# wyysf-98/MoCo_Flow

Hardware: AMD Instinct MI355X
Metric: ray-samples/sec (4096 rays x 64 samples) (higher is better)
Workload: dtype f32; 1 GPU; C2 NeRF 8x256 fp32 4096x64; rays_per_gpu=4096, samples_per_ray=64, global_rays=4096, loss_allreduce=False, main_has_collective=False

## Files before the change

### moco_flow_amd/csrc/mf_layout.hpp

```cpp
#pragma once
#include "../../include/mocoflow_hip.h"
#include "mf_core.hpp"

namespace mf {

inline int64_t round_up(int64_t x, int64_t m) { return (x + m - 1) / m * m; }

inline int single_skip_layer(uint32_t skip_mask, int D) {
  int s = 0;
  for (int l = 1; l < D; ++l)
    if ((skip_mask >> l) & 1u) { if (s) return -1; s = l; }
  return s;
}

constexpr int kPackHidden = -1;
struct PackBlock {
  const float* src;
  int s_n, s_k;
  int kind;
  int steps;
  int split;
  int cols;
};

struct PackRegion {
  PackBlock blk[2];
  int tiles;
  int groups;
  int n_rows;
  int row_terms;
  long long dst_group0;
};

struct ResCopy { const float* src; int dst_off; int n; float scale = 1.f; };

struct PackJob {
  PackRegion reg[MF_MAX_LAYERS + 3];
  int n_regions;
  int bf16;
  int xyz_cols;
  int half;
  float wscale;
  long long total_groups;
  float* panels;
  float* poison;
  ResCopy res[2];
  int n_res, res_floats;
  float* resident;
  PackRegion& add(int tiles, int groups, const PackBlock& b0, const PackBlock& b1 = PackBlock{}) {
    PackRegion& R = reg[n_regions++];
    R = PackRegion{{b0, b1}, tiles, groups, 0, 0, total_groups};
    total_groups += (long long)groups * tiles;
    return R;
  }
};
static_assert(sizeof(PackJob) <= 2048, "pack_panels_kernel's argument block");

int launch_pack(const PackJob& job, hipStream_t st, const char* what);

inline bool nerf_layout(const mf_nerf_desc& d, NetLayout& L, int bf16 = 0) {
  L = NetLayout{};
  const bool x3 = bf16 == MF_PREC_BF16X3;
  L.bf16 = bf16 ? 1 : 0;
  if (d.W != 256 && d.W != 128) return false;
  if (d.D < 2 || d.D + 1 > MF_MAX_LAYERS) return false;
  if (d.in_channels_xyz < 3 || d.in_channels_xyz > 64) return false;
  if (d.extra_feat_type != MF_EXTRA_NONE && (d.extra_feat_dim < 1 || d.extra_feat_dim > 32)) return false;
  if (d.skip_mask & 1u) return false;
  if (d.skip_mask >> d.D) return false;
  L.W = d.W;
  L.NK = d.W / 16;
  L.NP = d.W / 32;
  L.n_trunk = d.D + 1;
  if (bf16 && d.W != 256) return false;
  L.emb_steps = bf16 ? kKsNerfXyz : kStepsNerfXyz;
  L.emb_split = x3 ? 1 : 0;
  L.hsplit_mask = x3 ? ((1u << (d.D + 2)) - 1u) & ~1u : 0u;
  L.terms = 2;
  L.emb_mask = 1u | d.skip_mask;
  L.relu_mask = (1u << d.D) - 1u;
  switch (d.extra_feat_type) {
    case MF_EXTRA_NONE: L.extra_steps = 0; break;
    case MF_EXTRA_IND: L.extra_steps = bf16 ? kKsInd : kStepsInd; if (d.extra_feat_dim < 1) return false; break;
    case MF_EXTRA_DIR: L.extra_steps = bf16 ? kKsDir : kStepsDir; if (d.extra_feat_dim < 3) return false; break;
    default: return false;
  }
  int off = 0;
  L.off_bias_trunk = off; off += L.n_trunk * L.W;
  L.off_bias_extra = off; off += L.W / 2;
  L.off_head_w = off; off += L.W;
  L.off_head_b = off; off += 4;
  L.off_rgb_w = off; off += 3 * (L.W / 2);
  L.off_rgb_b = off; off += 4;
  L.n_head = 1;
  L.head_tiles = bf16 == MF_PREC_BF16 ? 1 : 0;
  L.res_bytes = round_up((int64_t)off * 4, kGroupBytes);
  int64_t groups = 0;
  L.max_groups = 0;
  for (int l = 0; l < L.n_trunk; ++l) {
    if (l == L.n_trunk - 1) groups += nerf_sigma_groups(L);
    const int g = trunk_groups(L, l);
    groups += (int64_t)g * L.NP;
    if ((x3 ? panel_cap(g) : g) > L.max_groups) L.max_groups = x3 ? panel_cap(g) : g;
  }
  const int ge = extra_groups(L);
  groups += (int64_t)ge * (L.NP / 2);
  if ((x3 ? panel_cap(ge) : ge) > L.max_groups) L.max_groups = x3 ? panel_cap(ge) : ge;
  groups += nerf_rgb_groups(L);
  L.panel_bytes = groups * kGroupBytes;
  return true;
}

struct FoldLayout {
  int64_t panel_bytes;
  int64_t scratch_bytes;
  int64_t off_w, off_b;
  int64_t off_x;
};
inline bool nerf_fold_layout(const mf_nerf_desc& d, NetLayout& L, FoldLayout& F) {
  F = FoldLayout{};
  if (!nerf_layout(d, L, 0) || L.W != 256) return false;
  F.panel_bytes = L.panel_bytes - (int64_t)trunk_groups(L, L.n_trunk - 1) * L.NP * kGroupBytes -
                  (int64_t)(extra_groups(L) - fold_extra_groups(L)) * (L.NP / 2) * kGroupBytes;
  const int64_t wb_bytes = round_up(((int64_t)(L.W / 2) * L.W + L.W / 2) * 4, kGroupBytes);
  F.scratch_bytes = wb_bytes + (int64_t)(L.W / 2) * fold_ext_cols(L) * 4;
  F.off_w = L.res_bytes + F.panel_bytes;
  F.off_b = F.off_w + (int64_t)(L.W / 2) * L.W * 4;
  F.off_x = F.off_w + wb_bytes;
  return true;
}

inline bool nof_layout(const mf_nof_desc& d, NetLayout& L, int bf16 = 0, bool wide_ok = false) {
  L = NetLayout{};
  const bool x3 = bf16 == MF_PREC_BF16X3;
  L.bf16 = bf16 ? 1 : 0;
  if (d.W != 128 && !(wide_ok && !bf16 && d.W == 256)) return false;
  if (d.D < 2 || d.D > MF_MAX_LAYERS) return false;
  if (d.in_channels_xyz < 3 || d.in_channels_xyz > 33 || d.extra_feat_dim < 0 || d.extra_feat_dim > 33) return false;
  if ((d.skip_mask & 1u) || (d.skip_mask >> d.D)) return false;
  L.W = d.W;
  L.NK = d.W / 16;
  L.NP = d.W / 32;
  L.n_trunk = d.D;
  L.emb_steps = bf16 ? kKsNofXyz : kStepsNofIn;
  L.emb_split = bf16 ? 1 : 0;
  L.hsplit_mask = x3 ? ((1u << d.D) - 1u) & ~1u : 0u;
  L.terms = x3 ? kNofTermsX3 : 2;
  L.half = (x3 && kNofHalfX3) ? 1 : 0;
  L.head_tiles = bf16 == MF_PREC_BF16 ? 1 : 0;
  L.emb_mask = 1u | d.skip_mask;
  L.relu_mask = (1u << d.D) - 1u;
  L.extra_steps = -1;
  L.n_head = d.use_quat ? 9 : 3;
  int off = 0;
  L.off_bias_trunk = off; off += L.n_trunk * L.W;
  L.off_head_w = off; off += L.n_head * L.W;
  L.off_head_b = off; off += bf16 ? 32 : 12;
  L.res_bytes = round_up((int64_t)off * 4, kGroupBytes);
  int64_t groups = 0;
  L.max_groups = 0;
  for (int l = 0; l < L.n_trunk; ++l) {
    const int g = trunk_groups(L, l);
    groups += (int64_t)g * L.NP;
    if ((x3 ? panel_cap(g) : g) > L.max_groups) L.max_groups = x3 ? panel_cap(g) : g;
  }
  if (bf16) {
    groups += head_groups(L);
    if (head_groups(L) > L.max_groups) L.max_groups = head_groups(L);
  }
  L.panel_bytes = groups * kGroupBytes;
  L.n_emb_layers = __builtin_popcount(L.emb_mask);
  L.ind_bytes = bf16 ? round_up((int64_t)L.n_emb_layers * L.W * kNofIndCols * 4, kGroupBytes) : 0;
  return true;
}

}
```

### moco_flow_amd/csrc/mf_nets.hpp

```cpp
#pragma once
#include "mf_core.hpp"

namespace mf {

MF_D const char* first_panel(const NetDev& n) { return n.packed + n.L.res_bytes; }
MF_D int first_groups(const NetDev& n) { return trunk_groups(n.L, 0); }

MF_D NextLayer follow_of(const NetDev& n) {
  NextLayer f;
  f.groups = trunk_groups(n.L, 0);
  f.jump = n.packed + n.L.res_bytes;
  f.bias_off = n.res_lds + n.L.off_bias_trunk * 4;
  return f;
}
MF_D NextLayer next_trunk(const NetDev& n, int layer) {
  NextLayer f;
  f.groups = trunk_groups(n.L, layer);
  f.jump = nullptr;
  f.bias_off = n.res_lds + (n.L.off_bias_trunk + layer * n.L.W) * 4;
  return f;
}

MF_D NextLayer next_extra(const NetDev& n) {
  NextLayer f;
  f.groups = extra_groups(n.L);
  f.jump = nullptr;
  f.bias_off = n.res_lds + n.L.off_bias_extra * 4;
  return f;
}

MF_D void load_resident(const NetDev& n, const LaneId& id) {
  const int groups = (int)(n.L.res_bytes / kGroupBytes);
  for (int g = id.wave; g < groups; g += kWaves) blds16(n.packed, id.lane * 16, g * kGroupBytes, n.res_lds + g * kGroupBytes);
}

template <int PD>
MF_D void start_program(const NetDev& n, Stream& st, CarryT<PD>& carry, const LaneId& id) {
  st.start(first_panel(n), first_groups(n), id);
  carry.load(st.slot_off(0) + id.lane * 16, n.res_lds + n.L.off_bias_trunk * 4, id.g);
}

template <int NK, bool DUMP = false>
MF_D void extra_layer(const NetDev& net, const f32x4 (&act)[NK],
                      const float (&ext)[kStepsExtraMax], f32x4 (&out)[NK / 2],
                      Stream& st, CarryT<kPD>& carry, const LaneId& id, const NextLayer& nxt,
                      float* dump_row = nullptr, unsigned* mask_row = nullptr) {
  constexpr int NPO = NK / 4;
  constexpr int QH = NK;
  const int groups = extra_groups(net.L);
  const int qe = net.L.extra_steps / 4;
  const uint32_t bias_off = net.res_lds + net.L.off_bias_extra * 4;
  const float dummy[4] = {0.f, 0.f, 0.f, 0.f};
  static_assert(NPO % 4 == 0, "mask words collect four panels");
  unsigned macc = 0;
#pragma unroll
  for (int t = 0; t < NPO; ++t) {
    const uint32_t p = st.slot_off(0) + id.lane * 16;
    const uint32_t pn = st.slot_off(1) + id.lane * 16;
    const uint32_t nb = (t + 1 < NPO) ? bias_off + 32 * (t + 1) * 4 : nxt.bias_off;
    auto hook = [&](int ph) { st.template sync_and_dma<DUMP>(t + 2 < NPO ? groups : nxt.groups, t == NPO - 2 ? nxt.jump : nullptr, id, ph); };
    f32x4 E, O;
    out_pair<2, NK, 4>(carry, act, dummy, p, pn, nb, id.g, id.wave < kWaves / 2 && !(st.dbg & 64), hook,
                             -__builtin_inff(), E, O);
#pragma unroll
    for (int q = 0; q < kStepsExtraMax / 4; ++q) {
      if (q < qe) {
        const f32x4 wE = lds_f4(p + (2 * (QH + q)) * kGroupBytes);
        const f32x4 wO = lds_f4(p + (2 * (QH + q) + 1) * kGroupBytes);
#pragma unroll
        for (int r = 0; r < 4; ++r) {
          E = MF_MFMA(wE[r], ext[4 * q + r], E);
          O = MF_MFMA(wO[r], ext[4 * q + r], O);
        }
      }
    }
#pragma unroll
    for (int i = 0; i < 4; ++i) {
      E[i] = fmaxf(E[i], 0.f);
      O[i] = fmaxf(O[i], 0.f);
    }
    out[2 * t] = E;
    out[2 * t + 1] = O;
    if constexpr (DUMP) {
      if (dump_row) {
        *reinterpret_cast<f32x4*>(dump_row + 32 * t + 4 * id.g) = E;
        *reinterpret_cast<f32x4*>(dump_row + 32 * t + 16 + 4 * id.g) = O;
      }
      const bool wm = __ballot(mask_row != nullptr) != 0ull;
      const bool put = wm && relu_mask_put(macc, mask_row, dump_row && mask_row, t, id.g, E, O);
      st.keep2 = __ballot(dump_row != nullptr) != 0ull ? (put ? 3 : 2) : 0;
    }
    st.advance();
  }
}

MF_D NextLayer next_extra_fold(const NetDev& n, uint32_t bias_off) {
  NextLayer f;
  f.groups = fold_extra_groups(n.L);
  f.jump = nullptr;
  f.bias_off = bias_off;
  return f;
}
template <int NK>
MF_D void extra_layer_fold(const NetDev& net, const f32x4 (&act)[NK], f32x4 (&out)[NK / 2], uint32_t bias_off,
                           Stream& st, CarryT<kPD>& carry, const LaneId& id, const NextLayer& nxt) {
  constexpr int NPO = NK / 4;
  const int groups = fold_extra_groups(net.L);
  const float dummy[4] = {0.f, 0.f, 0.f, 0.f};
#pragma unroll
  for (int t = 0; t < NPO; ++t) {
    const uint32_t p = st.slot_off(0) + id.lane * 16;
    const uint32_t pn = st.slot_off(1) + id.lane * 16;
    const uint32_t nb = (t + 1 < NPO) ? bias_off + 32 * (t + 1) * 4 : nxt.bias_off;
    auto hook = [&](int ph) { st.sync_and_dma(t + 2 < NPO ? groups : nxt.groups, t == NPO - 2 ? nxt.jump : nullptr, id, ph); };
    out_pair<2, NK, 4>(carry, act, dummy, p, pn, nb, id.g, id.wave < kWaves / 2 && !(st.dbg & 64), hook, 0.f, out[2 * t],
                       out[2 * t + 1]);
    st.advance();
  }
}

constexpr int kLongPairs = 4;
MF_D int long_groups(const NetDev& n) { return kLongPairs * trunk_groups(n.L, 0); }
MF_D NextLayer follow_of_long(const NetDev& n) {
  NextLayer f = follow_of(n);
  f.groups = long_groups(n);
  return f;
}
template <int PD>
MF_D void start_program_long(const NetDev& n, Stream& st, CarryT<PD>& carry, const LaneId& id) {
  st.start(first_panel(n), long_groups(n), id);
  carry.load(st.slot_off(0) + id.lane * 16, n.res_lds + n.L.off_bias_trunk * 4, id.g);
}
template <int NK, int EMB>
MF_D void trunk_layer0_long(const NetDev& net, f32x4 (&act)[NK], const float (&emb)[EMB], Stream& st, CarryT<kPD>& carry,
                            const LaneId& id, const NextLayer& nxt) {
  constexpr int NP = NK / 2;
  static_assert(NP % kLongPairs == 0 && NP / kLongPairs == 2, "both long panels' DMA (two ahead) is the next layer's");
  constexpr uint32_t pair_bytes = 2 * (EMB / 4) * kGroupBytes;
  const float lo = (net.L.relu_mask & 1) ? 0.f : -__builtin_inff();
  const uint32_t bias_off = net.res_lds + net.L.off_bias_trunk * 4;
  const bool late = id.wave < kWaves / 2 && !(st.dbg & 64);
#pragma unroll
  for (int sp = 0; sp < NP / kLongPairs; ++sp) {
    const uint32_t p = st.slot_off(0) + id.lane * 16;
    const uint32_t pn = st.slot_off(1) + id.lane * 16;
#pragma unroll
    for (int i = 0; i < kLongPairs; ++i) {
      const int t = sp * kLongPairs + i;
      const uint32_t nb = (t + 1 < NP) ? bias_off + 32 * (t + 1) * 4 : nxt.bias_off;
      auto hook = [&](int ph) { if (i == (late ? kLongPairs / 2 : 0)) st.sync_and_dma(nxt.groups, nullptr, id, ph); };
      out_pair<1, NK, EMB>(carry, act, emb, p + i * pair_bytes, i + 1 < kLongPairs ? p + (i + 1) * pair_bytes : pn, nb, id.g, false,
                           hook, lo, act[2 * t], act[2 * t + 1]);
    }
    st.advance();
  }
}

template <int NK, bool DUMP = false, bool FOLD = false, bool LONG0 = false>
MF_D void nerf_eval(const NetDev& net, const float (&embx)[kStepsNerfXyz], const float (&ext)[kStepsExtraMax],
                    bool sigma_only, Stream& st, CarryT<kPD>& carry, const LaneId& id,
                    const NextLayer& follow, float& sigma, float (&rgb)[3], float* dump_row = nullptr,
                    unsigned* mask_row = nullptr, uint32_t ray_bias = 0) {
  f32x4 act[NK];
#pragma unroll
  for (int t = 0; t < NK; ++t)
#pragma unroll
    for (int i = 0; i < 4; ++i) act[t][i] = 0;
  static_assert(!(FOLD && DUMP), "the dump rows hold xyz_encoding_final's output");
  const int D = net.L.n_trunk - 1;
  for (int l = 0; l < D; ++l) {
    const bool last = sigma_only && l == D - 1;
    if constexpr (LONG0) {
      if (l == 0) {
        trunk_layer0_long<NK, kStepsNerfXyz>(net, act, embx, st, carry, id, next_trunk(net, 1));
        st.tl.stamp(10, id);
        continue;
      }
    }
    trunk_layer<NK, kStepsNerfXyz, DUMP>(net, l, act, embx, st, carry, id,
                                               last ? follow : ((FOLD && l == D - 1) ? next_extra_fold(net, ray_bias) : next_trunk(net, l + 1)),
                                               dump_row ? dump_row + l * net.L.W : nullptr, mask_row ? mask_row + l * 8 : nullptr);
    st.tl.stamp(10 + l, id);
  }
  float sg[1];
  valu_head(act, net.res_lds + net.L.off_head_w * 4, net.L.W, net.res_lds + net.L.off_head_b * 4, id.g, sg);
  sigma = sg[0];
  st.tl.stamp(30, id);
  if (sigma_only) return;
  if constexpr (!FOLD) {
    const NextLayer ex = next_extra(net);
    trunk_layer<NK, kStepsNerfXyz, DUMP>(net, D, act, embx, st, carry, id, ex,
                                               dump_row ? dump_row + D * net.L.W : nullptr);
  }
  st.tl.stamp(31, id);
  f32x4 e[NK / 2];
  if constexpr (FOLD) extra_layer_fold<NK>(net, act, e, ray_bias, st, carry, id, follow);
  else
  extra_layer<NK, DUMP>(net, act, ext, e, st, carry, id, follow, dump_row ? dump_row + (D + 1) * net.L.W : nullptr,
                        mask_row ? mask_row + (D + 1) * 8 : nullptr);
  st.tl.stamp(33, id);
  float o[3];
  valu_head(e, net.res_lds + net.L.off_rgb_w * 4, net.L.W / 2, net.res_lds + net.L.off_rgb_b * 4, id.g, o);
#pragma unroll
  for (int c = 0; c < 3; ++c) rgb[c] = 1.f / (1.f + expf(-o[c]));
}

template <bool FAST = false>
MF_D void quat_transform(const float (&T)[9], const float (&xyz)[3], float (&out)[3]) {
  const float vx = T[0], vy = T[1], vz = T[2];
  float qx, qy, qz, qw;
  if constexpr (FAST) {
    const float n = fmaxf(__builtin_amdgcn_sqrtf(vx * vx + vy * vy + vz * vz), 1e-8f);
    const float rev = n * 0.15915494309189535f;
    const float s_n = __builtin_amdgcn_sinf(rev) * __builtin_amdgcn_rcpf(n);
    qx = vx * s_n; qy = vy * s_n; qz = vz * s_n; qw = __builtin_amdgcn_cosf(rev);
    const float rq = __builtin_amdgcn_rcpf(fmaxf(__builtin_amdgcn_sqrtf(qx * qx + qy * qy + qz * qz + qw * qw), 1e-12f));
    qx *= rq; qy *= rq; qz *= rq; qw *= rq;
  } else {
    float n = sqrtf(vx * vx + vy * vy + vz * vz);
    n = fmaxf(n, 1e-8f);
    float sn, cn;
    sincosf(n, &sn, &cn);
    qx = vx * sn / n; qy = vy * sn / n; qz = vz * sn / n; qw = cn;
    const float qn = fmaxf(sqrtf(qx * qx + qy * qy + qz * qz + qw * qw), 1e-12f);
    qx /= qn; qy /= qn; qz /= qn; qw /= qn;
  }
  const float tx = 2.f * qx, ty = 2.f * qy, tz = 2.f * qz;
  const float twx = tx * qw, twy = ty * qw, twz = tz * qw;
  const float txx = tx * qx, txy = ty * qx, txz = tz * qx;
  const float tyy = ty * qy, tyz = tz * qy, tzz = tz * qz;
  const float R00 = 1.f - (tyy + tzz), R01 = txy - twz, R02 = txz + twy;
  const float R10 = txy + twz, R11 = 1.f - (txx + tzz), R12 = tyz - twx;
  const float R20 = txz - twy, R21 = tyz + twx, R22 = 1.f - (txx + tyy);
  const float px = xyz[0] - T[3], py = xyz[1] - T[4], pz = xyz[2] - T[5];
  out[0] = (px * R00 + py * R10 + pz * R20) + T[3] + T[6];
  out[1] = (px * R01 + py * R11 + pz * R21) + T[4] + T[7];
  out[2] = (px * R02 + py * R12 + pz * R22) + T[5] + T[8];
}

template <bool DUMP = false, int NK = 8>
MF_D void nof_eval(const NetDev& net, const float (&emb)[kStepsNofIn], const float (&xyz)[3], Stream& st,
                   CarryT<kPD>& carry, const LaneId& id, const NextLayer& follow, float (&out)[3],
                   float* drow = nullptr, bool masks = false) {
  static_assert(!DUMP || NK == 8, "the dump layout (bit rows: four words per layer) is the 128-wide one");
  f32x4 act[NK];
#pragma unroll
  for (int t = 0; t < NK; ++t)
#pragma unroll
    for (int i = 0; i < 4; ++i) act[t][i] = 0;
  const int D = net.L.n_trunk;
  for (int l = 0; l < D; ++l) {
    const bool last = l == D - 1;
    trunk_layer<NK, kStepsNofIn, DUMP>(net, l, act, emb, st, carry, id, last ? follow : next_trunk(net, l + 1),
                                       drow ? drow + l * net.L.W : nullptr,
                                       (DUMP && drow && masks) ? reinterpret_cast<unsigned*>(drow + D * net.L.W + 16) + 4 * l : nullptr);
  }
  const uint32_t wo = net.res_lds + net.L.off_head_w * 4, bo = net.res_lds + net.L.off_head_b * 4;
  float T[9] = {0.f, 0.f, 0.f, 0.f, 0.f, 0.f, 0.f, 0.f, 0.f};
  if (net.L.n_head == 9) {
    valu_head(act, wo, net.L.W, bo, id.g, T);
    quat_transform(T, xyz, out);
  } else {
    float T3[3];
    valu_head(act, wo, net.L.W, bo, id.g, T3);
#pragma unroll
    for (int c = 0; c < 3; ++c) { T[c] = T3[c]; out[c] = T3[c] + xyz[c]; }
  }
  if constexpr (DUMP) {
    if (drow && id.g == 0) {
      float4* tr = reinterpret_cast<float4*>(drow + D * net.L.W);
      tr[0] = make_float4(T[0], T[1], T[2], T[3]);
      tr[1] = make_float4(T[4], T[5], T[6], T[7]);
      tr[2] = make_float4(T[8], 0.f, 0.f, 0.f);
      tr[3] = make_float4(0.f, 0.f, 0.f, 0.f);
    }
  }
}

MF_D void nof_embed(float (&emb)[kStepsNofIn], const float (&xyz)[3], float ind, const EmbParams& exyz,
                    const EmbParams& eind, int g) {
  emb_eval<3, 5>(emb, xyz, exyz, g);
  const float iv[1] = {ind};
  emb_eval<1, 16>(emb + BlkXyz5::SLOTS, iv, eind, g);
#pragma unroll
  for (int e = BlkXyz5::SLOTS + BlkInd16::SLOTS; e < kStepsNofIn; ++e) emb[e] = 0.f;
}

MF_D void nof_embed_lds(float (&emb)[kStepsNofIn], const float (&xyz)[3], float ind, uint32_t par_xyz, uint32_t par_ind, int g) {
  emb_eval_lds<3, 5>(emb, xyz, par_xyz, g);
  const float iv[1] = {ind};
  emb_eval_lds<1, 16>(emb + BlkXyz5::SLOTS, iv, par_ind, g);
#pragma unroll
  for (int e = BlkXyz5::SLOTS + BlkInd16::SLOTS; e < kStepsNofIn; ++e) emb[e] = 0.f;
}

}
```

### moco_flow_amd/csrc/mf_pack.hip

```cpp
#include <hip/hip_fp16.h>
#include "mf_host.hpp"
#include "mf_layout.hpp"

namespace mf {

__device__ inline unsigned short bf16_rne(float x) {
  const unsigned u = __float_as_uint(x);
  const unsigned rnd = u + 0x7fffu + ((u >> 16) & 1u);
  return (unsigned short)(((u & 0x7f800000u) == 0x7f800000u ? u : rnd) >> 16);
}

__device__ inline float resident_value(const ResCopy* c, int n, int idx) {
  float v = 0.f;
  for (int k = 0; k < n; ++k) {
    const int o = idx - c[k].dst_off;
    if (o >= 0 && o < c[k].n) v = c[k].src[o] * c[k].scale;
  }
  return v;
}

__device__ inline float block_at(const PackBlock& B, int n, int c) {
  return (c >= 0 && c < B.cols) ? B.src[(long long)n * B.s_n + (long long)c * B.s_k] : 0.f;
}

__global__ void pack_panels_kernel(PackJob job) {
  const long long gidx = (long long)blockIdx.x * blockDim.x + threadIdx.x;
  if (gidx < job.res_floats) job.resident[gidx] = resident_value(job.res, job.n_res, (int)gidx);
  const long long grp = ((long long)blockIdx.x * blockDim.x + __builtin_amdgcn_readfirstlane(threadIdx.x)) >> 6;
  if (grp >= job.total_groups) return;
  const int lane = (int)(gidx & 63);
  int ri = 0;
  while (ri + 1 < job.n_regions && grp >= job.reg[ri + 1].dst_group0) ++ri;
  const PackRegion& R = job.reg[ri];
  const long long local = grp - R.dst_group0;
  const int P = (int)(local / R.groups), gi = (int)(local % R.groups);
  float4 v = make_float4(0.f, 0.f, 0.f, 0.f);
  float* pv = &v.x;
  if (job.bf16) {
    const int i = lane & 31, h = lane >> 5;
    int srow = 32 * P + i, rterm = 0;
    bool zero_row = R.n_rows && srow >= R.n_rows;
    if (R.row_terms) {
      zero_row = !(srow < R.n_rows || (srow >= R.row_terms && srow < R.row_terms + R.n_rows));
      if (srow >= R.row_terms) { rterm = 1; srow -= R.row_terms; }
    }
    const int g0 = R.blk[0].split * R.blk[0].steps;
    const PackBlock B = gi < g0 ? R.blk[0] : R.blk[1];
    const int gb = gi < g0 ? gi : gi - g0;
    unsigned short h8[8] = {0, 0, 0, 0, 0, 0, 0, 0};
    const bool half = job.half != 0;
    const float ws = job.wscale;
    bool sat = false;
    auto term = [half, ws, &sat](float w, int t) {
      if (half) {
        w = w * ws;
        if (!(fabsf(w) <= 65504.f)) sat = true;
        w = fminf(fmaxf(w, -65504.f), 65504.f);
        __half hb = __float2half_rn(w);
        if (t > 0) hb = __float2half_rn(w - __half2float(hb));
        return __half_as_ushort(hb);
      }
      unsigned short b = bf16_rne(w);
      for (int k = 0; k < t; ++k) {
        w -= __uint_as_float((unsigned)b << 16);
        b = bf16_rne(w);
      }
      return b;
    };
    if (!zero_row && gb < B.split * B.steps) {
      const int ks = gb / B.split, t = R.row_terms ? rterm : gb % B.split;
#pragma unroll
      for (int e = 0; e < 8; ++e) {
        const int c = B.kind == kPackHidden ? 16 * ks + hid_perm2(h, e) : emb_feature2(B.kind, h, 8 * ks + e, job.xyz_cols);
        h8[e] = term(block_at(B, srow, c), t);
      }
    }
    unsigned* pu = reinterpret_cast<unsigned*>(&v.x);
    for (int w = 0; w < 4; ++w) pu[w] = (unsigned)h8[2 * w] | ((unsigned)h8[2 * w + 1] << 16);
    reinterpret_cast<float4*>(job.panels)[gidx] = v;
    if (sat && job.poison) { job.poison[0] = __int_as_float(0x7fc00000); job.poison[4] = __int_as_float(0x7fc00000); }
    return;
  }
  const int b = gi >> 1, half = gi & 1;
  const int i = lane & 15, g = lane >> 4;
  const int n = 32 * P + 16 * half + i;
  const PackBlock B = b < R.blk[0].steps ? R.blk[0] : R.blk[1];
  const int q = b < R.blk[0].steps ? b : b - R.blk[0].steps;
  if (!(R.n_rows && n >= R.n_rows) && q < B.steps)
#pragma unroll
    for (int r = 0; r < 4; ++r)
      pv[r] = block_at(B, n, B.kind == kPackHidden ? 16 * q + 4 * g + r : emb_feature(B.kind, g, 4 * q + r, job.xyz_cols));
  reinterpret_cast<float4*>(job.panels)[gidx] = v;
}

struct ResJob { ResCopy c[2 * MF_MAX_LAYERS + 8]; int n; float* res; int total; };

__global__ void pack_resident_kernel(ResJob job) {
  const int idx = blockIdx.x * blockDim.x + threadIdx.x;
  if (idx >= job.total) return;
  job.res[idx] = resident_value(job.c, job.n, idx);
}

struct IndJob { const float* W[MF_MAX_LAYERS]; int n_in[MF_MAX_LAYERS]; int n_layers, rows, col0, cols; float* dst; float scale; };

__global__ void pack_ind_kernel(IndJob job) {
  const int idx = blockIdx.x * blockDim.x + threadIdx.x;
  const int per_layer = job.rows * kNofIndCols;
  if (idx >= job.n_layers * per_layer) return;
  const int e = idx / per_layer, r = (idx % per_layer) / kNofIndCols, c = idx % kNofIndCols;
  job.dst[(e * kNofIndCols + c) * job.rows + r] = c < job.cols ? job.scale * job.W[e][(long long)r * job.n_in[e] + job.col0 + c] : 0.f;
}

struct FoldJob { const float *We, *Wf, *be, *bf; int W, ld_e; float *Wp, *bp; float* Wx; int xcols, ext; };

__global__ void fold_final_kernel(FoldJob job) {
  const int idx = blockIdx.x * blockDim.x + threadIdx.x;
  const int half = job.W / 2;
  if (idx >= half * job.W) return;
  if (idx < half * job.xcols) {
    const int n = idx / job.xcols, c = idx % job.xcols;
    job.Wx[idx] = c < job.ext ? job.We[(long long)n * job.ld_e + job.W + c] : 0.f;
  }
  const int n = idx / job.W, k = idx % job.W;
  const float* we = job.We + (long long)n * job.ld_e;
  double acc = 0.0;
  for (int j = 0; j < job.W; ++j) acc += (double)we[j] * (double)job.Wf[(long long)j * job.W + k];
  job.Wp[idx] = (float)acc;
  if (idx < half) {
    const float* wb = job.We + (long long)idx * job.ld_e;
    double b = 0.0;
#ifndef MF_FOLD_BREAK_BIAS
    for (int j = 0; j < job.W; ++j) b += (double)wb[j] * (double)job.bf[j];
#endif
    job.bp[idx] = (float)((double)job.be[idx] + b);
  }
}

int launch_pack(const PackJob& job, hipStream_t st, const char* what) {
  const long long slots = job.total_groups * 64 > job.res_floats ? job.total_groups * 64 : job.res_floats;
  hipLaunchKernelGGL(pack_panels_kernel, dim3((unsigned)((slots + 255) / 256)), dim3(256), 0, st, job);
  return check_launch(what);
}

static int launch_pack(const PackJob& job, const ResJob& rj, hipStream_t st) {
  hipLaunchKernelGGL(pack_resident_kernel, dim3((rj.total + 255) / 256), dim3(256), 0, st, rj);
  return launch_pack(job, st, "mf_pack");
}

}

using namespace mf;

extern "C" int64_t mf_nerf_packed_bytes_p(const mf_nerf_desc* d, int32_t precision) {
  NetLayout L;
  if (!d || (precision < MF_PREC_F32 || precision > MF_PREC_BF16X3) || !nerf_layout(*d, L, precision)) { fail(MF_E_UNSUPPORTED, "mf_nerf_packed_bytes: unsupported NeRF configuration"); return 0; }
  return L.res_bytes + L.panel_bytes;
}

extern "C" int64_t mf_nof_packed_bytes_p(const mf_nof_desc* d, int32_t precision) {
  NetLayout L;
  if (!d || (precision < MF_PREC_F32 || precision > MF_PREC_BF16X3) || !nof_layout(*d, L, precision, precision == MF_PREC_F32)) { fail(MF_E_UNSUPPORTED, "mf_nof_packed_bytes: unsupported NoF configuration"); return 0; }
  return L.res_bytes + L.panel_bytes + L.ind_bytes;
}

static int32_t nerf_pack(const mf_nerf_desc* d, int32_t precision, void* packed, void* stream, bool fold) {
  NetLayout L;
  FoldLayout F{};
  if (!d || !packed) return fail(MF_E_INVALID, "mf_nerf_pack: null argument");
  if (precision < MF_PREC_F32 || precision > MF_PREC_BF16X3) return fail(MF_E_INVALID, "mf_nerf_pack: precision %d", precision);
  if (fold ? !nerf_fold_layout(*d, L, F) : !nerf_layout(*d, L, precision))
    return fail(MF_E_UNSUPPORTED, "mf_nerf_pack: unsupported NeRF configuration "
                                       "(W=%d D=%d in_channels_xyz=%d)", d->W, d->D, d->in_channels_xyz);
  const int64_t panel_bytes = fold ? F.panel_bytes : L.panel_bytes;
  float* const fold_w = fold ? reinterpret_cast<float*>(static_cast<char*>(packed) + F.off_w) : nullptr;
  float* const fold_b = fold ? reinterpret_cast<float*>(static_cast<char*>(packed) + F.off_b) : nullptr;
  PackJob job{};
  ResJob rj{};
  const int esplit = L.emb_split ? L.terms : 1, equad = L.bf16 ? 1 : 4;
  auto head_region = [&](const float* W, int rows, int groups) {
    PackRegion& R = job.add(1, groups, PackBlock{W, groups * 16, 1, kPackHidden, groups, 1, groups * 16});
    R.n_rows = rows;
    R.row_terms = 8;
  };
  for (int l = 0; l < L.n_trunk; ++l) {
    if (l == L.n_trunk - 1 && L.head_tiles) {
      if (!d->sigma_w) return fail(MF_E_INVALID, "mf_nerf_pack: missing sigma weight");
      head_region(d->sigma_w, 1, nerf_sigma_groups(L));
    }
    const bool has_emb = (L.emb_mask >> l) & 1;
    const float* W = l < d->D ? d->trunk_w[l] : d->final_w;
    if (!W) return fail(MF_E_INVALID, "mf_nerf_pack: missing weight pointer for layer %d", l);
    if (fold && l == d->D) continue;
    const int hid0 = has_emb ? d->in_channels_xyz : 0, n_in = hid0 + (l > 0 ? L.W : 0);
    job.add(L.NP, trunk_groups(L, l),
            PackBlock{W, n_in, 1, kEmbNerfXyz, has_emb ? L.emb_steps / equad : 0, esplit, d->in_channels_xyz},
            PackBlock{W + hid0, n_in, 1, kPackHidden, l > 0 ? hidden_batches(L) : 0, ((L.hsplit_mask >> l) & 1) ? L.terms : 1, L.W});
    const float* b = l < d->D ? d->trunk_b[l] : d->final_b;
    rj.c[rj.n++] = ResCopy{b, L.off_bias_trunk + l * L.W, L.W};
  }
  {
    const int ext = d->extra_feat_type == MF_EXTRA_NONE ? 0 : d->extra_feat_dim;
    const float* W = d->extra_w;
    if (!W) return fail(MF_E_INVALID, "mf_nerf_pack: missing extra_encoding weight");
    const int kind = d->extra_feat_type == MF_EXTRA_DIR ? kEmbDir : (d->extra_feat_type == MF_EXTRA_IND ? kEmbInd : kEmbNone);
    if (fold) job.add(L.NP / 2, fold_extra_groups(L), PackBlock{fold_w, L.W, 1, kPackHidden, hidden_batches(L), 1, L.W});
    else job.add(L.NP / 2, extra_groups(L),
                 PackBlock{W, L.W + ext, 1, kPackHidden, hidden_batches(L), ((L.hsplit_mask >> L.n_trunk) & 1) ? L.terms : 1, L.W},
                 PackBlock{W + L.W, L.W + ext, 1, kind, L.extra_steps / equad, esplit, ext});
    if (fold && (!d->extra_b || !d->final_b)) return fail(MF_E_INVALID, "mf_nerf_pack: missing bias pointer of the folded layers");
    rj.c[rj.n++] = ResCopy{fold ? fold_b : d->extra_b, L.off_bias_extra, L.W / 2};
  }
  if (L.head_tiles) {
    if (!d->rgb_w) return fail(MF_E_INVALID, "mf_nerf_pack: missing rgb weight");
    head_region(d->rgb_w, 3, nerf_rgb_groups(L));
  }
  rj.c[rj.n++] = ResCopy{d->sigma_w, L.off_head_w, L.W};
  rj.c[rj.n++] = ResCopy{d->sigma_b, L.off_head_b, 1};
  rj.c[rj.n++] = ResCopy{d->rgb_w, L.off_rgb_w, 3 * (L.W / 2)};
  rj.c[rj.n++] = ResCopy{d->rgb_b, L.off_rgb_b, 3};
  for (int k = 0; k < rj.n; ++k)
    if (!rj.c[k].src) return fail(MF_E_INVALID, "mf_nerf_pack: missing bias/head pointer (%d)", k);
  job.bf16 = L.bf16;
  job.xyz_cols = d->in_channels_xyz;
  job.panels = reinterpret_cast<float*>(static_cast<char*>(packed) + L.res_bytes);
  rj.res = static_cast<float*>(packed);
  rj.total = (int)(L.res_bytes / 4);
  if (job.total_groups * kGroupBytes != panel_bytes) return fail(MF_E_INVALID, "mf_nerf_pack: layout mismatch");
  if (fold) {
    const int ext = d->extra_feat_type == MF_EXTRA_NONE ? 0 : d->extra_feat_dim;
    const FoldJob fj{d->extra_w, d->final_w, d->extra_b, d->final_b, L.W, L.W + ext, fold_w, fold_b,
                     reinterpret_cast<float*>(static_cast<char*>(packed) + F.off_x), fold_ext_cols(L), ext};
    hipLaunchKernelGGL(fold_final_kernel, dim3((L.W / 2) * L.W / 256), dim3(256), 0, static_cast<hipStream_t>(stream), fj);
    if (int e = check_launch("mf_nerf_pack_fold")) return e;
  }
  return launch_pack(job, rj, static_cast<hipStream_t>(stream));
}

extern "C" int32_t mf_nerf_pack_p(const mf_nerf_desc* d, int32_t precision, void* packed, void* stream) {
  return nerf_pack(d, precision, packed, stream, false);
}

extern "C" int64_t mf_nerf_fold_packed_bytes(const mf_nerf_desc* d) {
  NetLayout L;
  FoldLayout F;
  if (!d || !nerf_fold_layout(*d, L, F)) { fail(MF_E_UNSUPPORTED, "mf_nerf_fold_packed_bytes: unsupported NeRF configuration (fp32, W = 256)"); return 0; }
  return L.res_bytes + F.panel_bytes + F.scratch_bytes;
}

extern "C" int32_t mf_nerf_pack_fold(const mf_nerf_desc* d, void* packed, void* stream) {
  return nerf_pack(d, MF_PREC_F32, packed, stream, true);
}

extern "C" int32_t mf_nof_pack_p(const mf_nof_desc* d, int32_t precision, void* packed, void* stream) {
  NetLayout L;
  if (!d || !packed) return fail(MF_E_INVALID, "mf_nof_pack: null argument");
  if (precision < MF_PREC_F32 || precision > MF_PREC_BF16X3) return fail(MF_E_INVALID, "mf_nof_pack: precision %d", precision);
  if (!nof_layout(*d, L, precision, precision == MF_PREC_F32)) return fail(MF_E_UNSUPPORTED, "mf_nof_pack: unsupported NoF configuration "
                                      "(W=%d D=%d in_channels_xyz=%d extra_feat_dim=%d)", d->W, d->D,
                                      d->in_channels_xyz, d->extra_feat_dim);
  PackJob job{};
  ResJob rj{};
  const int cin = d->in_channels_xyz + d->extra_feat_dim;
  const float wscale = L.half ? (float)(1 << kNofHalfSW) : 1.f, bscale = L.half ? (float)(1 << (kNofHalfSA + kNofHalfSW)) : 1.f;
  const int esplit = L.emb_split ? L.terms : 1, equad = L.bf16 ? 1 : 4;
  for (int l = 0; l < L.n_trunk; ++l) {
    const bool has_emb = (L.emb_mask >> l) & 1;
    const float* W = d->trunk_w[l];
    if (!W || !d->trunk_b[l]) return fail(MF_E_INVALID, "mf_nof_pack: missing parameter pointer for layer %d", l);
    const int hid0 = has_emb ? cin : 0, n_in = hid0 + (l > 0 ? L.W : 0);
    job.add(L.NP, trunk_groups(L, l),
            PackBlock{W, n_in, 1, kEmbNofIn, has_emb ? L.emb_steps / equad : 0, esplit, cin},
            PackBlock{W + hid0, n_in, 1, kPackHidden, l > 0 ? hidden_batches(L) : 0, ((L.hsplit_mask >> l) & 1) ? L.terms : 1, L.W});
    rj.c[rj.n++] = ResCopy{d->trunk_b[l], L.off_bias_trunk + l * L.W, L.W, bscale};
  }
  if (!d->head_w || !d->head_b) return fail(MF_E_INVALID, "mf_nof_pack: missing head parameters");
  if (L.bf16) {
    PackRegion& R = job.add(1, head_groups(L), PackBlock{d->head_w, L.W, 1, kPackHidden, L.NK, L.head_tiles ? 1 : L.terms, L.W});
    R.n_rows = L.n_head;
    R.row_terms = L.head_tiles ? 16 : 0;
  }
  rj.c[rj.n++] = ResCopy{d->head_w, L.off_head_w, L.n_head * L.W};
  rj.c[rj.n++] = ResCopy{d->head_b, L.off_head_b, L.n_head, bscale};
  job.bf16 = L.bf16;
  job.xyz_cols = d->in_channels_xyz;
  job.half = L.half;
  job.wscale = wscale;
  job.panels = reinterpret_cast<float*>(static_cast<char*>(packed) + L.res_bytes);
  job.poison = L.half ? static_cast<float*>(packed) + L.off_head_b + 27 : nullptr;
  rj.res = static_cast<float*>(packed);
  rj.total = (int)(L.res_bytes / 4);
  if (job.total_groups * kGroupBytes != L.panel_bytes) return fail(MF_E_INVALID, "mf_nof_pack: layout mismatch");
  if (L.bf16) {
    IndJob ij{};
    for (int l = 0; l < L.n_trunk; ++l)
      if ((L.emb_mask >> l) & 1) {
        ij.W[ij.n_layers] = d->trunk_w[l];
        ij.n_in[ij.n_layers] = cin + (l > 0 ? L.W : 0);
        ++ij.n_layers;
      }
    ij.rows = L.W; ij.col0 = d->in_channels_xyz; ij.cols = d->extra_feat_dim;
    ij.scale = bscale;
    ij.dst = reinterpret_cast<float*>(static_cast<char*>(packed) + L.res_bytes + L.panel_bytes);
    const int total = ij.n_layers * ij.rows * kNofIndCols;
    hipLaunchKernelGGL(pack_ind_kernel, dim3((total + 255) / 256), dim3(256), 0, static_cast<hipStream_t>(stream), ij);
  }
  return launch_pack(job, rj, static_cast<hipStream_t>(stream));
}

extern "C" int64_t mf_nerf_packed_bytes(const mf_nerf_desc* d) { return mf_nerf_packed_bytes_p(d, MF_PREC_F32); }
extern "C" int64_t mf_nof_packed_bytes(const mf_nof_desc* d) { return mf_nof_packed_bytes_p(d, MF_PREC_F32); }
extern "C" int32_t mf_nerf_pack(const mf_nerf_desc* d, void* packed, void* stream) { return mf_nerf_pack_p(d, MF_PREC_F32, packed, stream); }
extern "C" int32_t mf_nof_pack(const mf_nof_desc* d, void* packed, void* stream) { return mf_nof_pack_p(d, MF_PREC_F32, packed, stream); }
```

### moco_flow_amd/csrc/mf_render.hip

```cpp
#include <cstddef>

#include "mf_host.hpp"
#include "mf_layout.hpp"
#include "mf_nets.hpp"
#include "mf_plan.hpp"
#include "mf_raypass.hpp"

namespace mf {

struct RenderParams {
  const float* rays; long long ray_stride; long long n_rays;
  const float* bg;
  int S;
  const float* z_vals; const float* z_steps; int use_disp;
  const float* noise;
  int activation, flags;
  NetDev nerf;
  int extra_type;
  NetDev bw, fw;
  float emb_par[4][32];
  uint32_t par_off;
  float *rgb, *depth, *opacity, *weights, *alphas, *disp_local, *disp_global;
  int G;
  long long n_groups;
  uint32_t ring_off, buf_bytes, sbuf_off, zbuf_off;
  int dbg;
  float* dump_acts; long long dump_stride; float* dump_rgbsigma; float* dump_xyz;
  unsigned* dump_mask; long long dump_mask_stride;
  float* dump_nof_acts; long long dump_nof_stride; float* dump_nof_emb; float* dump_nof_out;
  uint32_t nof_plane_pack;
};
struct FoldRenderParams : RenderParams {
  const float* fold_wx; int fold_xcols;
  uint32_t rbias_off;
};
constexpr int kRayPeFloats = 32;
constexpr int kFoldHalf = 128;

template <bool MOCO, bool DUMP>
__global__ __launch_bounds__(kThreads, 2) void render_kernel(RenderParams p) {
  constexpr bool FOLD = false;
#define MF_BODY_FOLD 0
#include "mf_render_body.hpp"
#undef MF_BODY_FOLD
}

template <bool MOCO>
__global__ __launch_bounds__(kThreads, 2) void render_fold_kernel(FoldRenderParams p) {
  constexpr bool DUMP = false, FOLD = true;
#define MF_BODY_FOLD 1
#include "mf_render_body.hpp"
#undef MF_BODY_FOLD
}

int render_pass_bf16(const mf_render_args* a, hipStream_t st, bool prepare_only);
int64_t render_workspace_bytes_bf16(const mf_render_args* a);

}

using namespace mf;

extern "C" int64_t mf_render_workspace_bytes(const mf_render_args* a) {
  if (!a || (a->precision != MF_PREC_BF16 && a->precision != MF_PREC_BF16X3) || a->n_rays <= 0) return 0;
  return render_workspace_bytes_bf16(a);
}

extern "C" int32_t mf_nof_emb_slot_features(int32_t* features80) {
  if (!features80) return fail(MF_E_INVALID, "mf_nof_emb_slot_features: null argument");
  for (int g = 0; g < 4; ++g)
    for (int e = 0; e < kStepsNofIn; ++e) features80[kStepsNofIn * g + e] = emb_feature(kEmbNofIn, g, e, 33);
  return MF_OK;
}

static int32_t check_render_args(const mf_render_args* a, NetLayout (&L)[3]) {
  if (!a->rays || a->ray_stride < 9) return fail(MF_E_INVALID, "mf_render_pass: rays missing or ray_stride < 9");
  if (!a->z_vals && !a->z_steps) return fail(MF_E_INVALID, "mf_render_pass: need z_vals or z_steps");
  if (a->activation != MF_ACT_RELU && a->activation != MF_ACT_SOFTPLUS)
    return fail(MF_E_INVALID, "mf_render_pass: activation %d not supported", a->activation);
  if (a->precision < MF_PREC_F32 || a->precision > MF_PREC_BF16X3)
    return fail(MF_E_INVALID, "mf_render_pass: precision %d", a->precision);
  if (!nerf_layout(*a->nerf, L[0], 0)) return fail(MF_E_UNSUPPORTED, "mf_render_pass: unsupported NeRF configuration");
  if (L[0].NK != 16) return fail(MF_E_UNSUPPORTED, "mf_render_pass: only W=256 NeRF is built");
  const bool dump = a->dump_acts || a->dump_rgbsigma || a->dump_xyz || a->dump_nof_acts;
  if (dump && a->precision == MF_PREC_BF16)
    return fail(MF_E_UNSUPPORTED, "mf_render_pass: the activation dump (training forward) exists in fp32 and in bf16x3");
  if (a->flags & MF_F_FOLDED_FINAL) {
    if (a->precision != MF_PREC_F32)
      return fail(MF_E_UNSUPPORTED, "mf_render_pass: MF_F_FOLDED_FINAL is built for MF_PREC_F32 (precision %d)", a->precision);
    if (dump || a->dump_mask || a->dump_nof_emb || a->dump_nof_out)
      return fail(MF_E_INVALID, "mf_render_pass: MF_F_FOLDED_FINAL with a dump_* pointer (the training forward reads mf_nerf_pack's stream)");
  }
  if (int e = check_xyz_embedding("mf_render_pass", a->emb_xyz, 10)) return e;
  const bool sigma_only = a->flags & MF_F_SIGMA_ONLY;
  if (!sigma_only && a->nerf->extra_feat_type == MF_EXTRA_DIR &&
      (a->emb_extra.in_channels != 3 || a->emb_extra.n_freqs > 4 ||
       3 * (2 * a->emb_extra.n_freqs + 1) > a->nerf->extra_feat_dim))
    return fail(MF_E_UNSUPPORTED, "mf_render_pass: dir embedding must have 3 channels, <= 4 frequencies and fit extra_feat_dim");
  if (!sigma_only && a->nerf->extra_feat_type == MF_EXTRA_IND &&
      (a->emb_extra.in_channels != 1 || a->emb_extra.n_freqs > 2 ||
       (2 * a->emb_extra.n_freqs + 1) > a->nerf->extra_feat_dim))
    return fail(MF_E_UNSUPPORTED, "mf_render_pass: ind embedding must have 1 channel, <= 2 frequencies and fit extra_feat_dim");
  const bool moco = a->nof_bw != nullptr;
  const bool chains = a->flags & (MF_F_CHAIN_LOCAL | MF_F_CHAIN_GLOBAL);
  if (!moco && chains) return fail(MF_E_INVALID, "mf_render_pass: chain flags need NoF models");
  if ((a->flags & MF_F_CHAIN_GLOBAL) && !(a->flags & MF_F_CHAIN_LOCAL))
    return fail(MF_E_INVALID, "mf_render_pass: chain_global without chain_local (the reference raises UnboundLocalError, rendering.py:276-280)");
  if ((a->flags & MF_F_CHAIN_GLOBAL) && a->ray_stride < 10)
    return fail(MF_E_INVALID, "mf_render_pass: chain_global needs the chained image index column (ray_stride >= 10)");
  if (moco) {
    if (!a->nof_bw_packed) return fail(MF_E_INVALID, "mf_render_pass: nof_bw_packed missing");
    if (!nof_layout(*a->nof_bw, L[1], 0)) return fail(MF_E_UNSUPPORTED, "mf_render_pass: unsupported backward NoF configuration");
    if (chains) {
      if (!a->nof_fw || !a->nof_fw_packed) return fail(MF_E_INVALID, "mf_render_pass: chain flags need the forward NoF");
      if (!nof_layout(*a->nof_fw, L[2], 0)) return fail(MF_E_UNSUPPORTED, "mf_render_pass: unsupported forward NoF configuration");
    }
    if (int e = check_nof_embeddings("mf_render_pass", a->nof_emb_xyz, a->nof_emb_ind)) return e;
  }
  return MF_OK;
}

static int32_t render_pass_f32(const mf_render_args* a, const NetLayout (&L)[3], hipStream_t st) {
  const bool moco = a->nof_bw != nullptr;
  const bool chains = a->flags & (MF_F_CHAIN_LOCAL | MF_F_CHAIN_GLOBAL);
  FoldRenderParams p{};
  fill_render_io(p, a);
  p.dbg = debug_flags();
  LdsPlan plan;
  auto place = [&](NetDev& n, const NetLayout& l, const void* packed) { n.L = l; plan.place(n, packed); };
  place(p.nerf, L[0], a->nerf_packed);
  emb_table(a->emb_xyz, p.emb_par[0], p.emb_par[0] + 16);
  emb_table(a->emb_extra, p.emb_par[1], p.emb_par[1] + 16);
  if (moco) {
    place(p.bw, L[1], a->nof_bw_packed);
    if (chains) place(p.fw, L[2], a->nof_fw_packed);
    emb_table(a->nof_emb_xyz, p.emb_par[2], p.emb_par[2] + 16);
    emb_table(a->nof_emb_ind, p.emb_par[3], p.emb_par[3] + 16);
  }
  p.par_off = plan.place_tables();
  plan.ring(p.ring_off, p.buf_bytes);
  uint32_t lds = plan.lds;

  FoldLayout F{};
  NetLayout Lf;
  const bool ray_table = (a->flags & MF_F_FOLDED_FINAL) && !(a->flags & MF_F_SIGMA_ONLY) &&
                         a->nerf->extra_feat_type != MF_EXTRA_NONE && nerf_fold_layout(*a->nerf, Lf, F);
  uint32_t ray_bytes = ray_table ? (kFoldHalf + kRayPeFloats) * 4 : 0;
  const bool home_row = ray_table && lds < kRenderLdsCap && (long long)a->n_samples * 20 + ray_bytes > (long long)(kRenderLdsCap - lds);
  if (home_row) ray_bytes = 0;
  if (int e = plan_ray_groups(a->n_rays, a->n_samples, kTile, lds, p.G, p.n_groups, ray_bytes)) return e;
  if (home_row) { p.G = 1; p.n_groups = a->n_rays; }
  place_sample_buffers(p, lds);
  if (ray_table) {
    static_assert((kFoldHalf + kRayPeFloats) <= 2 * kFoldHalf, "one row and one encoding fit a W-float bias slot");
    p.fold_wx = reinterpret_cast<const float*>(static_cast<const char*>(a->nerf_packed) + F.off_x);
    p.fold_xcols = fold_ext_cols(Lf);
    if (home_row) p.rbias_off = p.nerf.res_lds + (uint32_t)(p.nerf.L.off_bias_trunk + (p.nerf.L.n_trunk - 1) * p.nerf.L.W) * 4;
    else { p.rbias_off = lds; lds += (uint32_t)p.G * ray_bytes; }
  }

  if (int e = check_dump_rows(a, p.nerf.L)) return e;
  if (int e = check_dump_mask(a, p.nerf.L)) return e;
  if (a->dump_nof_acts) {
    if (!moco || !a->dump_nof_emb || !a->dump_nof_out) return fail(MF_E_INVALID, "mf_render_pass: dump_nof_acts needs NoF models, dump_nof_emb and dump_nof_out");
    if (a->dump_nof_stride < (int64_t)p.bw.L.n_trunk * p.bw.L.W + 16 || (a->dump_nof_stride & 3))
      return fail(MF_E_INVALID, "mf_render_pass: dump_nof_stride %lld invalid", (long long)a->dump_nof_stride);
    if (a->nof_fw && (p.fw.L.n_trunk != p.bw.L.n_trunk || p.fw.L.W != p.bw.L.W))
      return fail(MF_E_UNSUPPORTED, "mf_render_pass: NoF dumps need bw and fw of the same depth and width");
    if (int e = nof_plane_pack(a, p.nof_plane_pack)) return e;
  }
  p.dump_nof_acts = a->dump_nof_acts; p.dump_nof_stride = a->dump_nof_stride; p.dump_nof_emb = a->dump_nof_emb; p.dump_nof_out = a->dump_nof_out;
  const bool dump = a->dump_acts || a->dump_rgbsigma || a->dump_xyz || a->dump_nof_acts;
  if (!dump && (a->flags & MF_F_FOLDED_FINAL))
    return launch_lds(moco ? render_fold_kernel<true> : render_fold_kernel<false>, persistent_grid(p.n_groups), kThreads, lds, st, p,
                      "mf_render_pass", "mf_render_pass");
  void (*kern)(RenderParams) = dump ? (moco ? render_kernel<true, true> : render_kernel<false, true>)
                                    : (moco ? render_kernel<true, false> : render_kernel<false, false>);
  return launch_lds(kern, persistent_grid(p.n_groups), kThreads, lds, st, static_cast<const RenderParams&>(p), "mf_render_pass",
                    "mf_render_pass");
}

static int32_t render_entry(const mf_render_args* a, void* stream, bool prepare_only) {
  if (!a || !a->nerf || !a->nerf_packed) return fail(MF_E_INVALID, "mf_render_pass: null argument");
  if (a->n_rays < 0 || a->n_samples < 1) return fail(MF_E_INVALID, "mf_render_pass: n_rays=%lld n_samples=%d", (long long)a->n_rays, a->n_samples);
  if (a->n_rays == 0) return MF_OK;
  NetLayout L[3];
  if (int e = check_render_args(a, L)) return e;
  if (a->precision != MF_PREC_F32) return render_pass_bf16(a, static_cast<hipStream_t>(stream), prepare_only);
  return prepare_only ? MF_OK : render_pass_f32(a, L, static_cast<hipStream_t>(stream));
}
extern "C" int32_t mf_render_pass(const mf_render_args* a, void* stream) { return render_entry(a, stream, false); }
extern "C" int32_t mf_render_prepare(const mf_render_args* a, void* stream) { return render_entry(a, stream, true); }
```

Measured before the change: 137.3 million ray-samples/s.

## Split folded skip layers into embedding and hidden panel regions to shrink LDS ring

In the folded NeRF path, skip-connection layers are packed as two separate regions (embedding panels, then hidden panels). The kernel runs them as two passes, the second seeded with the first pass's partial sums. This lowers the maximum panel group count per stream slot, so the LDS ring buffer needs less space and more rays can be resident per block. The cost is a second pass over the accumulators on skip layers, extra sync/DMA points, a larger pack argument block, and more complex LDS planning that keeps the old budget envelope for choosing the home-row mode.

```diff
diff --git a/moco_flow_amd/csrc/mf_layout.hpp b/moco_flow_amd/csrc/mf_layout.hpp
--- a/moco_flow_amd/csrc/mf_layout.hpp
+++ b/moco_flow_amd/csrc/mf_layout.hpp
@@ -35,7 +35,7 @@
 struct ResCopy { const float* src; int dst_off; int n; float scale = 1.f; };
 
 struct PackJob {
-  PackRegion reg[MF_MAX_LAYERS + 3];
+  PackRegion reg[2 * MF_MAX_LAYERS + 2];
   int n_regions;
   int bf16;
   int xyz_cols;
@@ -54,7 +54,7 @@
     return R;
   }
 };
-static_assert(sizeof(PackJob) <= 2048, "pack_panels_kernel's argument block");
+static_assert(sizeof(PackJob) <= 4096, "pack_panels_kernel's argument block");
 
 int launch_pack(const PackJob& job, hipStream_t st, const char* what);
 
@@ -112,6 +112,7 @@
 }
 
 struct FoldLayout {
+  int max_groups;
   int64_t panel_bytes;
   int64_t scratch_bytes;
   int64_t off_w, off_b;
@@ -122,6 +123,7 @@
   if (!nerf_layout(d, L, 0) || L.W != 256) return false;
   F.panel_bytes = L.panel_bytes - (int64_t)trunk_groups(L, L.n_trunk - 1) * L.NP * kGroupBytes -
                   (int64_t)(extra_groups(L) - fold_extra_groups(L)) * (L.NP / 2) * kGroupBytes;
+  F.max_groups = 2 * hidden_batches(L) > 4 * trunk_groups(L, 0) ? 2 * hidden_batches(L) : 4 * trunk_groups(L, 0);
   const int64_t wb_bytes = round_up(((int64_t)(L.W / 2) * L.W + L.W / 2) * 4, kGroupBytes);
   F.scratch_bytes = wb_bytes + (int64_t)(L.W / 2) * fold_ext_cols(L) * 4;
   F.off_w = L.res_bytes + F.panel_bytes;
diff --git a/moco_flow_amd/csrc/mf_nets.hpp b/moco_flow_amd/csrc/mf_nets.hpp
--- a/moco_flow_amd/csrc/mf_nets.hpp
+++ b/moco_flow_amd/csrc/mf_nets.hpp
@@ -132,13 +132,12 @@
   carry.load(st.slot_off(0) + id.lane * 16, n.res_lds + n.L.off_bias_trunk * 4, id.g);
 }
 template <int NK, int EMB>
-MF_D void trunk_layer0_long(const NetDev& net, f32x4 (&act)[NK], const float (&emb)[EMB], Stream& st, CarryT<kPD>& carry,
-                            const LaneId& id, const NextLayer& nxt) {
+MF_D void emb_panels_long(const NetDev& net, int layer, f32x4 (&dst)[NK], const f32x4 (&hid)[NK], const float (&emb)[EMB], float lo,
+                          Stream& st, CarryT<kPD>& carry, const LaneId& id, const NextLayer& nxt, int tag0) {
   constexpr int NP = NK / 2;
   static_assert(NP % kLongPairs == 0 && NP / kLongPairs == 2, "both long panels' DMA (two ahead) is the next layer's");
   constexpr uint32_t pair_bytes = 2 * (EMB / 4) * kGroupBytes;
-  const float lo = (net.L.relu_mask & 1) ? 0.f : -__builtin_inff();
-  const uint32_t bias_off = net.res_lds + net.L.off_bias_trunk * 4;
+  const uint32_t bias_off = net.res_lds + (net.L.off_bias_trunk + layer * net.L.W) * 4;
   const bool late = id.wave < kWaves / 2 && !(st.dbg & 64);
 #pragma unroll
   for (int sp = 0; sp < NP / kLongPairs; ++sp) {
@@ -148,12 +147,79 @@
     for (int i = 0; i < kLongPairs; ++i) {
       const int t = sp * kLongPairs + i;
       const uint32_t nb = (t + 1 < NP) ? bias_off + 32 * (t + 1) * 4 : nxt.bias_off;
-      auto hook = [&](int ph) { if (i == (late ? kLongPairs / 2 : 0)) st.sync_and_dma(nxt.groups, nullptr, id, ph); };
-      out_pair<1, NK, EMB>(carry, act, emb, p + i * pair_bytes, i + 1 < kLongPairs ? p + (i + 1) * pair_bytes : pn, nb, id.g, false,
-                           hook, lo, act[2 * t], act[2 * t + 1]);
+      auto hook = [&](int ph) {
+        if (i == (late ? kLongPairs / 2 : 0)) {
+          st.tl.stamp(tag0 + 2 * sp, id);
+          st.sync_and_dma(nxt.groups, nullptr, id, ph);
+          st.tl.stamp(tag0 + 1 + 2 * sp, id);
+        }
+      };
+      out_pair<1, NK, EMB>(carry, hid, emb, p + i * pair_bytes, i + 1 < kLongPairs ? p + (i + 1) * pair_bytes : pn, nb, id.g, false,
+                           hook, lo, dst[2 * t], dst[2 * t + 1]);
     }
     st.advance();
   }
+}
+template <int NK, int EMB>
+MF_D void trunk_layer0_long(const NetDev& net, f32x4 (&act)[NK], const float (&emb)[EMB], Stream& st, CarryT<kPD>& carry,
+                            const LaneId& id, const NextLayer& nxt) {
+  emb_panels_long<NK, EMB>(net, 0, act, act, emb, (net.L.relu_mask & 1) ? 0.f : -__builtin_inff(), st, carry, id, nxt, 20);
+}
+
+MF_D bool fold_split_layer(const NetLayout& L, int layer) { return layer > 0 && ((L.emb_mask >> layer) & 1); }
+template <bool LONG>
+MF_D NextLayer next_trunk_fold(const NetDev& n, int layer) {
+  NextLayer f = next_trunk(n, layer);
+  if (fold_split_layer(n.L, layer)) f.groups = LONG ? long_groups(n) : trunk_groups(n.L, 0);
+  else f.groups = 2 * hidden_batches(n.L);
+  return f;
+}
+template <int MODE, bool SEEDED, int NK, int EMB>
+MF_D void fold_panels(const NetDev& net, int layer, const f32x4 (&act)[NK], f32x4 (&out)[NK], const float (&emb)[EMB], float lo,
+                      int groups, Stream& st, CarryT<kPD>& carry, const LaneId& id, const NextLayer& nxt) {
+  constexpr int NP = NK / 2;
+  const uint32_t bias_off = net.res_lds + (net.L.off_bias_trunk + layer * net.L.W) * 4;
+  const bool late = id.wave < kWaves / 2 && !(st.dbg & 64);
+#pragma unroll
+  for (int t = 0; t < NP; ++t) {
+    const uint32_t p = st.slot_off(0) + id.lane * 16;
+    const uint32_t pn = st.slot_off(1) + id.lane * 16;
+    const uint32_t nb = (t + 1 < NP) ? bias_off + 32 * (t + 1) * 4 : nxt.bias_off;
+    auto hook = [&](int ph) { st.sync_and_dma(t + 2 < NP ? groups : nxt.groups, t == NP - 2 ? nxt.jump : nullptr, id, ph); };
+    if constexpr (SEEDED) { carry.bE = out[2 * t]; carry.bO = out[2 * t + 1]; }
+    out_pair<MODE, NK, EMB>(carry, act, emb, p, pn, nb, id.g, late, hook, lo, out[2 * t], out[2 * t + 1]);
+    st.advance();
+  }
+}
+template <int NK, int EMB, bool LONG>
+MF_D void skip_layer_split(const NetDev& net, int layer, f32x4 (&act)[NK], const float (&emb)[EMB], Stream& st, CarryT<kPD>& carry,
+                           const LaneId& id, const NextLayer& nxt) {
+  const int hg = 2 * hidden_batches(net.L);
+  const float lo = ((net.L.relu_mask >> layer) & 1) ? 0.f : -__builtin_inff();
+  f32x4 out[NK];
+  NextLayer hidden;
+  hidden.groups = hg;
+  hidden.jump = nullptr;
+  hidden.bias_off = net.res_lds + (net.L.off_bias_trunk + layer * net.L.W) * 4;
+#ifdef MF_FOLD_BREAK_SKIP_SEED
+  constexpr bool seeded = false;
+#else
+  constexpr bool seeded = true;
+#endif
+  if constexpr (LONG) emb_panels_long<NK, EMB>(net, layer, out, act, emb, -__builtin_inff(), st, carry, id, hidden, 24);
+  else fold_panels<1, false, NK, EMB>(net, layer, act, out, emb, -__builtin_inff(), trunk_groups(net.L, 0), st, carry, id, hidden);
+  fold_panels<2, seeded, NK, EMB>(net, layer, act, out, emb, lo, hg, st, carry, id, nxt);
+#pragma unroll
+  for (int t = 0; t < NK; ++t) act[t] = out[t];
+}
+template <int NK, int EMB>
+MF_D void hidden_layer_fold(const NetDev& net, int layer, f32x4 (&act)[NK], const float (&emb)[EMB], Stream& st, CarryT<kPD>& carry,
+                            const LaneId& id, const NextLayer& nxt) {
+  f32x4 out[NK];
+  fold_panels<2, false, NK, EMB>(net, layer, act, out, emb, ((net.L.relu_mask >> layer) & 1) ? 0.f : -__builtin_inff(),
+                                 2 * hidden_batches(net.L), st, carry, id, nxt);
+#pragma unroll
+  for (int t = 0; t < NK; ++t) act[t] = out[t];
 }
 
 template <int NK, bool DUMP = false, bool FOLD = false, bool LONG0 = false>
@@ -170,12 +236,16 @@
   const int D = net.L.n_trunk - 1;
   for (int l = 0; l < D; ++l) {
     const bool last = sigma_only && l == D - 1;
-    if constexpr (LONG0) {
+    if constexpr (FOLD) {
+      const NextLayer nxt = last ? follow : (l == D - 1 ? next_extra_fold(net, ray_bias) : next_trunk_fold<LONG0>(net, l + 1));
       if (l == 0) {
-        trunk_layer0_long<NK, kStepsNerfXyz>(net, act, embx, st, carry, id, next_trunk(net, 1));
-        st.tl.stamp(10, id);
-        continue;
-      }
+        if constexpr (LONG0) trunk_layer0_long<NK, kStepsNerfXyz>(net, act, embx, st, carry, id, nxt);
+        else fold_panels<1, false, NK, kStepsNerfXyz>(net, 0, act, act, embx, (net.L.relu_mask & 1) ? 0.f : -__builtin_inff(),
+                                                      trunk_groups(net.L, 0), st, carry, id, nxt);
+      } else if (fold_split_layer(net.L, l)) skip_layer_split<NK, kStepsNerfXyz, LONG0>(net, l, act, embx, st, carry, id, nxt);
+      else hidden_layer_fold<NK, kStepsNerfXyz>(net, l, act, embx, st, carry, id, nxt);
+      st.tl.stamp(10 + l, id);
+      continue;
     }
     trunk_layer<NK, kStepsNerfXyz, DUMP>(net, l, act, embx, st, carry, id,
                                                last ? follow : ((FOLD && l == D - 1) ? next_extra_fold(net, ray_bias) : next_trunk(net, l + 1)),
diff --git a/moco_flow_amd/csrc/mf_pack.hip b/moco_flow_amd/csrc/mf_pack.hip
--- a/moco_flow_amd/csrc/mf_pack.hip
+++ b/moco_flow_amd/csrc/mf_pack.hip
@@ -192,9 +192,12 @@
     if (!W) return fail(MF_E_INVALID, "mf_nerf_pack: missing weight pointer for layer %d", l);
     if (fold && l == d->D) continue;
     const int hid0 = has_emb ? d->in_channels_xyz : 0, n_in = hid0 + (l > 0 ? L.W : 0);
-    job.add(L.NP, trunk_groups(L, l),
-            PackBlock{W, n_in, 1, kEmbNerfXyz, has_emb ? L.emb_steps / equad : 0, esplit, d->in_channels_xyz},
-            PackBlock{W + hid0, n_in, 1, kPackHidden, l > 0 ? hidden_batches(L) : 0, ((L.hsplit_mask >> l) & 1) ? L.terms : 1, L.W});
+    const PackBlock emb_blk{W, n_in, 1, kEmbNerfXyz, has_emb ? L.emb_steps / equad : 0, esplit, d->in_channels_xyz};
+    const PackBlock hid_blk{W + hid0, n_in, 1, kPackHidden, l > 0 ? hidden_batches(L) : 0, ((L.hsplit_mask >> l) & 1) ? L.terms : 1, L.W};
+    if (fold && has_emb && l > 0) {
+      job.add(L.NP, 2 * emb_blk.steps, emb_blk);
+      job.add(L.NP, 2 * hid_blk.steps, PackBlock{}, hid_blk);
+    } else job.add(L.NP, trunk_groups(L, l), emb_blk, hid_blk);
     const float* b = l < d->D ? d->trunk_b[l] : d->final_b;
     rj.c[rj.n++] = ResCopy{b, L.off_bias_trunk + l * L.W, L.W};
   }
diff --git a/moco_flow_amd/csrc/mf_render.hip b/moco_flow_amd/csrc/mf_render.hip
--- a/moco_flow_amd/csrc/mf_render.hip
+++ b/moco_flow_amd/csrc/mf_render.hip
@@ -127,7 +127,12 @@
   p.dbg = debug_flags();
   LdsPlan plan;
   auto place = [&](NetDev& n, const NetLayout& l, const void* packed) { n.L = l; plan.place(n, packed); };
+  FoldLayout F{};
+  NetLayout Lf;
+  const bool folded = (a->flags & MF_F_FOLDED_FINAL) && nerf_fold_layout(*a->nerf, Lf, F);
+  const int unfolded_groups = L[0].max_groups;
   place(p.nerf, L[0], a->nerf_packed);
+  if (folded) { p.nerf.L.max_groups = F.max_groups; plan.max_groups = F.max_groups; }
   emb_table(a->emb_xyz, p.emb_par[0], p.emb_par[0] + 16);
   emb_table(a->emb_extra, p.emb_par[1], p.emb_par[1] + 16);
   if (moco) {
@@ -140,12 +145,14 @@
   plan.ring(p.ring_off, p.buf_bytes);
   uint32_t lds = plan.lds;
 
-  FoldLayout F{};
-  NetLayout Lf;
-  const bool ray_table = (a->flags & MF_F_FOLDED_FINAL) && !(a->flags & MF_F_SIGMA_ONLY) &&
-                         a->nerf->extra_feat_type != MF_EXTRA_NONE && nerf_fold_layout(*a->nerf, Lf, F);
+  const bool ray_table = folded && !(a->flags & MF_F_SIGMA_ONLY) && a->nerf->extra_feat_type != MF_EXTRA_NONE;
   uint32_t ray_bytes = ray_table ? (kFoldHalf + kRayPeFloats) * 4 : 0;
-  const bool home_row = ray_table && lds < kRenderLdsCap && (long long)a->n_samples * 20 + ray_bytes > (long long)(kRenderLdsCap - lds);
+  const uint32_t lds_env = lds + (folded && plan.max_groups < unfolded_groups ? 3u * (uint32_t)(unfolded_groups - plan.max_groups) * kGroupBytes : 0u);
+  if (lds_env != lds) {
+    int g_env; long long n_env;
+    if (int e = plan_ray_groups(a->n_rays, a->n_samples, kTile, lds_env, g_env, n_env, 0)) return e;
+  }
+  const bool home_row = ray_table && lds_env < kRenderLdsCap && (long long)a->n_samples * 20 + ray_bytes > (long long)(kRenderLdsCap - lds_env);
   if (home_row) ray_bytes = 0;
   if (int e = plan_ray_groups(a->n_rays, a->n_samples, kTile, lds, p.G, p.n_groups, ray_bytes)) return e;
   if (home_row) { p.G = 1; p.n_groups = a->n_rays; }
```

Result: no change. 137.7 million ray-samples/s, median of 6 (+0.3%).
